# carlozamu/dynamic-video-compression-surveillance

Hardware: AMD Instinct MI355X
Metric: Mpixels/s (frames/s × H×W) 1080p frame-diff path @1/2/4/8 GPU; % HBM roofline (higher is better)
Workload: dtype u8; 1 GPU; fd_1080p_single_feed_per_gpu; width=1920, height=1080, feeds_per_gpu=1, io=device, ring_frames=384, noisy=False, in_format=BGR, out_format=BGR, launch=batched, frames_per_launch=383, output_sets=2, parallelism=feed-per-gpu x1

## Files before the change

dynamic-video-compression-surveillance_amd/_native.py:

```python
from __future__ import annotations

import ctypes
import glob
import os
import shutil
import subprocess

PKG_DIR = os.path.dirname(os.path.abspath(__file__))
CSRC = os.path.join(PKG_DIR, "csrc")
LIB_PATH = os.path.join(PKG_DIR, "libdvc_hip.so")
HIPCC_FLAGS = ["--offload-arch=gfx950", "-O3", "-std=c++17", "-fPIC", "-shared", "-ffp-contract=off"]

DVC_OK = 0
DVC_E_INVALID, DVC_E_HIP, DVC_E_STATE, DVC_E_NOMEM, DVC_E_UNSUPPORTED = -1, -2, -3, -4, -5
DVC_E_ODD_DCT = -6
DVC_FLAG_DEVICE_PTRS = 0x1
DVC_FLAG_KTIMING = 0x2
DVC_FLAG_KEEP_PLANES = 0x4
DVC_FLAG_JOIN_STREAM = 0x8
DVC_FLAG_OF_DIRECT_SUMS = 0x10
DVC_FLAG_OUT_I420 = 0x20
DVC_FLAG_FD_UNFUSED = 0x40
KTIME_OUT, KTIME_FRONT_FUSED = 0, 1
KTIME_FLOW, KTIME_FLOW_SCAN, KTIME_FLOW_SCAN2 = 2, 3, 4
FMT_BGR, FMT_I420, FMT_NV12 = 0, 1, 2
FMT_GRAY = 3
FORMATS = {"BGR": FMT_BGR, "I420": FMT_I420, "NV12": FMT_NV12}

PLANE_GRAY, PLANE_MOTION, PLANE_FILTERED, PLANE_ACC, PLANE_DILATED = range(5)
OF_PLANE_RAW, OF_PLANE_SMOOTH, OF_PLANE_MORPH, OF_PLANE_RECT, OF_PLANE_GRAY = range(5)

ABI_VERSION = 10
MAX_BATCH = 512


class DvcError(RuntimeError):

    def __init__(self, code: int, msg: str):
        super().__init__(f"dvc error {code}: {msg}")
        self.code = code


class FdParams(ctypes.Structure):
    _fields_ = [
        ("width", ctypes.c_int32),
# ... 470 lines not shown
```

dynamic-video-compression-surveillance_amd/csrc/fd_api.hip:

```cpp
#include <hip/hip_runtime.h>
#include <cstdlib>

#include <cmath>
#include <cstdio>
#include <algorithm>
#include <cstring>
#include <utility>
#include <vector>

#include "../../include/dvc.h"
#include "fd_kernels.h"
#include "klaunch.h"
#include "host_common.h"
#include "yuv_kernels.h"
#include "tune.h"

using dvc_host::fail;
using dvc_host::dct_matrix;
using dvc_host::gauss_taps;

struct FdGraph {
    std::vector<dvc::KNode> rec[4];
    std::vector<hipGraphNode_t> node[4];
    hipGraph_t g = nullptr;
// ... 397 lines not shown
    if (p.flags & DVC_FLAG_KEEP_PLANES) {
        if ((e = h->mem.alloc(&h->dbg_dil, 8 * H * WW)) != hipSuccess) return bad(e, "hipMalloc");
    }
    if (!(p.flags & DVC_FLAG_DEVICE_PTRS)) {
        const size_t Fi = (size_t)h->sip * h->sh * mb, Fo = 3 * N * (size_t)mb;
        for (Stage& st : h->stage) {
            if ((e = h->mem.alloc(&st.d_in, Fi)) != hipSuccess) return bad(e, "hipMalloc");
            if ((e = h->mem.alloc(&st.d_ov, Fo)) != hipSuccess) return bad(e, "hipMalloc");
            if ((e = h->mem.alloc(&st.d_cp, Fo)) != hipSuccess) return bad(e, "hipMalloc");
            if ((e = h->mem.alloc_pinned(&st.h_in, Fi)) != hipSuccess) return bad(e, "hipHostMalloc");
            if ((e = h->mem.alloc_pinned(&st.h_ov, Fo)) != hipSuccess) return bad(e, "hipHostMalloc");
            if ((e = h->mem.alloc_pinned(&st.h_cp, Fo)) != hipSuccess) return bad(e, "hipHostMalloc");
            for (hipEvent_t* ev : {&st.ev_h2d, &st.ev_d2h, &st.ev_free})
                if ((e = h->mem.event(ev)) != hipSuccess) return bad(e, "hipEventCreate");
        }
        if ((e = h->mem.alloc_pinned(&h->h_acc, N)) != hipSuccess) return bad(e, "hipHostMalloc");
    }
    if ((e = hipMemsetAsync(h->stats, 0, 8 * 4 * 64, h->stream)) != hipSuccess) return bad(e, "hipMemset");
    if ((e = hipMemsetAsync(h->err, 0xff, 8, h->stream)) != hipSuccess) return bad(e, "hipMemset");
    if ((e = hipMemsetAsync(h->acc, 0, accb, h->stream)) != hipSuccess) return bad(e, "hipMemset");
    {
        size_t sz[dvc::CclBufs::NARR];
        dvc::CclBufs::sizes(h->g, mb, sz);
        if ((e = hipMemsetAsync(h->slot[0].c.gpar, 0, sz[6], h->stream)) != hipSuccess) return bad(e, "hipMemset");
    }
    if ((e = hipStreamSynchronize(h->stream)) != hipSuccess) return bad(e, "hipStreamSynchronize");
    *out = h;
    return DVC_OK;
}

}

static int stage_input(dvc_fd* h, Slot& S, const uint8_t* src, size_t pitch, size_t fstride, int n,
                       const uint8_t** d, int* dp, size_t* dfs, int crows, dvc::SrcFmt* sf)
{
    if (sf) *sf = dvc::SrcFmt{DVC_FMT_BGR, 0, 0, 0};
    const int direct = in_place(h, src, pitch, fstride, n);
    if (direct == 1) {
        *d = src;
        *dp = (int)pitch;
        *dfs = fstride;
        return DVC_OK;
    }
    if (sf && direct == 2) {
        const dvc::YuvLayout L = dvc::yuv_layout(src, pitch, h->fmt, crows, fstride);
        *sf = dvc::SrcFmt{h->fmt, L.uoff, L.voff, L.cpitch};
        *d = src;
// ... 96 lines not shown
{
    if (n <= S.gc_frames) return DVC_OK;
    int cap = 1;
    while (cap < n) cap *= 2;
    cap = std::min(cap, std::min(h->max_batch, GRAPH_OWN_CCL_FRAMES));
    if (!S.gc_mem.dev.empty()) {
        if (S.recorded) HIP_OK(hipEventSynchronize(S.ev_out));
        S.gc_mem.free_all();
        S.gc_frames = 0;
    }
    size_t sz[dvc::CclBufs::NARR];
    dvc::CclBufs::sizes(h->g, cap, sz);
    S.gc = S.c;
    void** ptrs[dvc::CclBufs::NARR];
    S.gc.ptrs(ptrs);
    for (int i = 0; i < dvc::CclBufs::NARR; ++i) {
        if (!dvc::CclBufs::working_set(i)) continue;
        const hipError_t e = S.gc_mem.alloc(ptrs[i], sz[i]);
        if (e != hipSuccess) {
            S.gc_mem.free_all();
            return dvc_host::create_failed(e, "graph contour-filter set");
        }
    }
    HIP_OK(hipMemsetAsync(S.gc.gpar, 0, sz[6], graph_stream(h, (int)(&S - h->slot))));
    S.gc_frames = cap;
    return DVC_OK;
}

static int enqueue_graph(dvc_fd* h, Slot& S, std::vector<dvc::KNode> (&rec)[4], const std::vector<hipEvent_t>& wait_out,
                         bool shared)
{
    const int k = (int)(h->seq % NSLOT);
    Slot& P = h->slot[(h->seq + NSLOT - 1) % NSLOT];
    hipStream_t z = graph_stream(h, k);
    const hipEvent_t ccl_ev = P.recorded && P.graph && !P.shared_ccl ? P.ev_acc : P.ev_ccl;
    FdGraph* G = nullptr;
    for (FdGraph& x : S.graphs) {
        bool same = x.shared == shared;
        for (int sg = 0; sg < 4 && same; ++sg) {
            same = x.rec[sg].size() == rec[sg].size();
            for (size_t u = 0; same && u < rec[sg].size(); ++u) same = x.rec[sg][u].same_shape(rec[sg][u]);
        }
        if (same) {
            G = &x;
            break;
        }
    }
// ... 202 lines not shown
    a.n = n;
    a.ksize = h->p.ksize;
    a.anchor = h->p.anchor;
    a.alpha = h->p.alpha;
    a.beta = h->p.beta;
    a.gamma = h->p.gamma;
    a.quant = h->p.quant;
    a.qinv = 1.0 / (double)h->p.quant;
    {
        const float z = std::rint(std::fmaf(0.0f, h->p.alpha, std::fmaf(0.0f, h->p.beta, h->p.gamma)));
        a.acc0_fixed = z < 0.5f && z > -0.5f;
        const float dil1 = std::fmaf(255.0f, h->p.beta, h->p.gamma);
        static const bool acc_general = dvc::tune_env("DVC_ACC_GENERAL") != nullptr;
        a.acc_fast = dvc::acc_fast_ok(h->p.alpha, h->p.beta, h->p.gamma) && !acc_general;
        std::memcpy(&a.dil1_bits, &dil1, 4);
    }
    a.M = h->M;
    a.Mtab = h->Mtab;
    a.stats = h->stats;
    a.dbg_dil = h->dbg_dil;
    a.err = h->err;
    a.frame0 = h->frames;
    h->last_fused = fused;
    if (graph) {
        std::vector<dvc::KNode> rec[4];
        hipError_t e[4];
        hipStream_t z = graph_stream(h, (int)(h->seq % NSLOT));
        const bool shared = n > GRAPH_OWN_CCL_FRAMES;
        if (!shared) {
            rc = graph_ccl(h, S, n);
            if (rc) return rc;
        }
        dvc::g_krec = &rec[0];
        e[0] = dvc::launch_front(d, dp, dfs, sf, n, h->gray[h->gcur], h->gray[h->gcur ^ 1], h->gs, S.c.mbits, h->g,
                                 h->p.ithresh, z, fused ? &fo : nullptr);
        dvc::g_krec = &rec[1];
        e[1] = dvc::launch_ccl(shared ? S.c : S.gc, h->g, n, h->p.min_area2, z);
        dvc::g_krec = &rec[2];
        e[2] = dvc::launch_accumulate(a, z);
        dvc::g_krec = &rec[3];
        e[3] = dvc::launch_out(a, z, fused);
        dvc::g_krec = nullptr;
        for (hipError_t x : e) HIP_OK(x);
        rc = enqueue_graph(h, S, rec, wait_out, shared);
        if (rc) return rc;
        h->prev_graph = true;
        S.graph = true;
        S.shared_ccl = shared;
    } else {
        if (timed) {
            while (h->ev.size() < h->ev_used + 2) {
                hipEvent_t e;
                HIP_OK(hipEventCreate(&e));
                h->ev.push_back(e);
            }
        }
        if (timed && fused) HIP_OK(hipEventRecord(h->ev[h->ev_used], h->s_front));
        if (!(skip & 1))
            HIP_OK(dvc::launch_front(d, dp, dfs, sf, n, h->gray[h->gcur], h->gray[h->gcur ^ 1], h->gs, S.c.mbits, h->g,
                                     h->p.ithresh, h->s_front, fused ? &fo : nullptr));
        if (timed && fused) {
            HIP_OK(hipEventRecord(h->ev[h->ev_used + 1], h->s_front));
            h->ev_used += 2;
        }
        HIP_OK(hipEventRecord(S.ev_front, h->s_front));
        HIP_OK(hipStreamWaitEvent(s_ccl, S.ev_front, 0));
        if (S.recorded) HIP_OK(hipStreamWaitEvent(s_ccl, S.ev_acc, 0));
        if (!(skip & 2)) HIP_OK(dvc::launch_ccl(S.c, h->g, n, h->p.min_area2, s_ccl));
        HIP_OK(hipEventRecord(S.ev_ccl, s_ccl));
        HIP_OK(hipStreamWaitEvent(h->s_acc, S.ev_ccl, 0));
        if (S.recorded) HIP_OK(hipStreamWaitEvent(h->s_acc, S.ev_out, 0));
        if (!(skip & 4)) HIP_OK(dvc::launch_accumulate(a, h->s_acc));
        HIP_OK(hipEventRecord(S.ev_acc, h->s_acc));
        HIP_OK(hipStreamWaitEvent(h->s_out, S.ev_acc, 0));
        if (timed && !fused) HIP_OK(hipEventRecord(h->ev[h->ev_used], h->s_out));
        if (!(skip & 8)) HIP_OK(dvc::launch_out(a, h->s_out, fused));
        if (timed && !fused) {
            HIP_OK(hipEventRecord(h->ev[h->ev_used + 1], h->s_out));
            h->ev_used += 2;
        }
        HIP_OK(hipEventRecord(S.ev_out, h->s_out));
        h->prev_graph = false;
        S.graph = false;
        S.shared_ccl = true;
    }
    h->gcur ^= 1;
    S.recorded = true;
    h->seq++;
    h->frames += (uint64_t)n;
    h->last_n = n;
    return DVC_OK;
}

static int drain_stage(dvc_fd* h, Stage& st)
{
// ... 212 lines not shown
    if (width < 4 || height < 4 || width > 65520)
        return fail(DVC_E_INVALID, "mask %dx%d: sides must be 4..65520", width, height);
    HIP_OK(hipSetDevice(device));
    dvc::RowGeom g{width, height, (width + 63) / 64, width / 2 + 1};
    const size_t W = width, H = height, WW = g.WW;
    std::vector<uint64_t> bits(H * WW, 0);
    for (size_t y = 0; y < H; ++y)
        for (size_t x = 0; x < W; ++x)
            if (mask[y * W + x]) bits[y * WW + x / 64] |= 1ull << (x % 64);
    dvc::CclBufs c{};
    size_t sz[dvc::CclBufs::NARR];
    void** ptrs[dvc::CclBufs::NARR];
    dvc::CclBufs::sizes(g, 1, sz);
    c.ptrs(ptrs);
    unsigned long long* stats = nullptr;
    dvc_host::DevMem mem;
    hipError_t e = mem.alloc(&stats, 8 * 4 * 64);
    for (int i = 0; i < dvc::CclBufs::NARR && e == hipSuccess; ++i) e = mem.alloc(ptrs[i], sz[i]);
    if (e != hipSuccess) return fail(DVC_E_NOMEM, "hipMalloc failed");
    c.stats = stats;
    hipStream_t s = nullptr;
    e = hipMemcpy(c.mbits, bits.data(), 8 * H * WW, hipMemcpyHostToDevice);
    if (e == hipSuccess) e = hipMemset(stats, 0, 8 * 4 * 64);
    if (e == hipSuccess) e = hipMemset(c.gpar, 0, sz[6]);
    if (e == hipSuccess) e = dvc::launch_ccl(c, g, 1, min_area2, s);
    if (e == hipSuccess) e = hipDeviceSynchronize();
    unsigned long long st[4];
    if (e == hipSuccess) e = dvc_host::fold_stats(stats, st);
    if (e == hipSuccess) e = dvc_host::read_bit_plane(c.kbits, W, H, WW, filtered);
    if (e != hipSuccess) return fail(DVC_E_HIP, "contour filter: %s", hipGetErrorString(e));
    if (components) *components = st[2];
    return DVC_OK;
}

}
```

dynamic-video-compression-surveillance_amd/csrc/fd_kernels.h:

```cpp
#pragma once
#include <hip/hip_runtime.h>
#include <stdint.h>

namespace dvc {

struct RowGeom {
    int W, H;
    int WW;
    int CAP;
};

struct GaussTaps {
    int n;
    uint16_t t[64];
};

struct alignas(8) DctMat {
    float m[64];
    float mt[64];
};

struct CclBufs {
    uint64_t* mbits;
    uint64_t* fbits;
    uint16_t *rs, *re;
    uint32_t* nfg;
    uint32_t* fpar;
    uint32_t* gpar;
    uint8_t* gE;
    uint32_t* area2;
    uint64_t* kbits;
    unsigned long long* stats;
    uint8_t* kocc = nullptr;
    int kfull = 0;
    uint32_t* rowb = nullptr;
    static size_t rowb_bytes(const RowGeom& g, size_t frames) { return (size_t)8 * g.H * frames; }

    __host__ __device__ static size_t bits_per_frame(const RowGeom& g) { return (size_t)g.H * g.WW; }
    __host__ __device__ CclBufs frame(size_t f, const RowGeom& g) const
    {
        const size_t nb = (size_t)g.H * g.WW, nr = (size_t)g.H * g.CAP, ng = (size_t)g.H * (g.CAP + 1);
        return CclBufs{mbits + f * nb, fbits + f * nb, rs + f * nr, re + f * nr, nfg + f * g.H, fpar + f * nr,
                       gpar + f * (ng + 1), gE + f * ng, area2 + f * nr, kbits + f * nb, stats,
                       kocc ? kocc + f * g.H : nullptr, kfull, rowb + f * 2 * g.H};
    }
    static constexpr int NARR = 11;
    static void sizes(const RowGeom& g, size_t frames, size_t out[NARR])
    {
        const size_t nb = (size_t)g.H * g.WW, nr = (size_t)g.H * g.CAP, ng = (size_t)g.H * (g.CAP + 1);
        const size_t s[NARR] = {8 * nb, 8 * nb, 2 * nr, 2 * nr, 4 * (size_t)g.H, 4 * nr, 4 * (ng + 1), ng, 4 * nr, 8 * nb,
                                rowb_bytes(g, 1)};
        for (int i = 0; i < NARR; ++i) out[i] = s[i] * frames;
    }
    void ptrs(void** out[NARR])
    {
        void** p[NARR] = {(void**)&mbits, (void**)&fbits, (void**)&rs,    (void**)&re,    (void**)&nfg, (void**)&fpar,
                          (void**)&gpar,  (void**)&gE,    (void**)&area2, (void**)&kbits, (void**)&rowb};
        for (int i = 0; i < NARR; ++i) out[i] = p[i];
    }
    static bool working_set(int i) { return (i >= 1 && i <= 8) || i == 10; }
};

struct SrcFmt {
    int fmt;
    size_t uoff, voff, cpitch;
};

struct BackArgs {
    RowGeom g;
    const uint8_t* bgr;
    int pitch;
    size_t fstride;
    SrcFmt sf;
    uint8_t* acc;
    int ap;
    uint8_t* overlay;
    uint8_t* compressed;
    int opitch;
    size_t ostride;
    int obytes;
    int out_i420;
    const uint64_t* kbits;
    const uint8_t* kocc;
// ... 32 lines not shown
    size_t ostride;
    float quant;
    double qinv;
    DctMat M;
    int B;
    int i420;
};
hipError_t launch_front(const uint8_t* bgr, int pitch, size_t fstride, const SrcFmt& sf, int n, const uint8_t* gray_in,
                        uint8_t* gray_out, int gs, uint64_t* mbits, const RowGeom& g, int ithresh, hipStream_t s,
                        const FrontOut* fo = nullptr);
struct ResizeTab {
    int sw, sh, dw, dh;
    int area2x;
    int simd_end;
    const int* xo;
    const int* yo;
};
void resize_tables(int sw, int sh, int dw, int dh, int* host_x , int* host_y , int* area2x,
                   int* simd_end);
hipError_t launch_resize(const uint8_t* src, int spitch, size_t sstride, uint8_t* dst, int dpitch, size_t dstride,
                         int n, const ResizeTab& t, hipStream_t s);
int band_rows(const RowGeom& g);
size_t ccl_max_lds(const RowGeom& g);
hipError_t launch_ccl(const CclBufs& c, const RowGeom& g, int n, int64_t min_area2, hipStream_t s);
hipError_t launch_accumulate(const BackArgs& a, hipStream_t s);
inline bool acc_fast_ok(float alpha, float beta, float gamma)
{
    const float d0 = __builtin_fmaf(0.0f, beta, gamma), d1 = __builtin_fmaf(255.0f, beta, gamma);
    uint32_t d0b;
    __builtin_memcpy(&d0b, &d0, 4);
    return d0b == 0 && alpha >= 0.0f && alpha <= 1.0f && d1 >= 0.0f && d1 <= 255.0f &&
           __builtin_rintf(__builtin_fmaf(255.0f, alpha, d1)) <= 255.0f;
}
hipError_t launch_out(const BackArgs& a, hipStream_t s, bool fix = false);
inline bool fast_block(int B) { return B == 4 || B == 8; }

}
```

dynamic-video-compression-surveillance_amd/csrc/fd_kernels.hip:

```cpp
#include <hip/hip_runtime.h>
#include <stdint.h>

#include <algorithm>
#include <cmath>
#include <cstdlib>
#include <cstring>

#include "dvc_device.h"
#include "fd_kernels.h"
#include "klaunch.h"
#include "dct_const.h"
#include "yuv_px.h"
#include "../../include/dvc.h"
#include "tune.h"

namespace dvc {

thread_local std::vector<KNode>* g_krec = nullptr;

__global__ void __launch_bounds__(256) k_gray(const uint8_t* __restrict__ bgr, int pitch,
                                              uint8_t* __restrict__ gray, int W, int H, int gs)
{
    int q = blockIdx.x * 256 + threadIdx.x;
    int y = blockIdx.y;
// ... 763 lines not shown
        const uint32_t base = fb.rowb[2 * y];
        const uint8_t* ge = gE + (fb.rowb[2 * y + 1] - 1);
        for (int k = sl; k < n; k += CG) {
            const uint32_t root = fpar[base + k];
            if (!((int64_t)area2[root] > min_area2)) continue;
            const int e = re[base + k];
            paint_bits(s_k, 0, g.WW, rs[base + k], e);
            if (k + 1 < n && !ge[k + 1]) paint_bits(s_k, 0, g.WW, e + 1, (int)rs[base + k + 1] - 1);
        }
    }
    wave_sync_lds();
    unsigned long long any = 0;
    if (act)
        for (int w = sl; w < g.WW; w += CG) any |= s_k[w];
    for (int d = 1; d < CG; d <<= 1) any |= __shfl_xor(any, d, CG);
    if (act && (any || !fb.kocc || fb.kfull))
        for (int w = sl; w < g.WW; w += CG) kbits[(size_t)y * g.WW + w] = s_k[w];
    if (act && sl == 0 && fb.kocc) fb.kocc[y] = any ? 1 : 0;
}

template <int CG>
__global__ void __launch_bounds__(256) k_resolve(CclBufs cb, RowGeom g)
{
    const CclBufs fb = cb.frame(blockIdx.y, g);
    const uint16_t* __restrict__ rs = fb.rs;
    const uint16_t* __restrict__ re = fb.re;
    const uint32_t* __restrict__ nfg = fb.nfg;
    uint32_t* fpar = fb.fpar;
    uint32_t* gpar = fb.gpar;
    uint8_t* __restrict__ gE = fb.gE;
    const uint64_t* __restrict__ mbits = fb.mbits;
    uint64_t* __restrict__ fbits = fb.fbits;
    extern __shared__ __attribute__((aligned(16))) unsigned long long lds_r[];
    const int slot = threadIdx.x / CG, sl = threadIdx.x & (CG - 1);
    const int y = blockIdx.x * cg_rows<CG>() + slot;
    const bool act = y < g.H;
    unsigned long long* s_f = lds_r + (size_t)slot * g.WW;
    const int n = act ? (int)nfg[y] : 0;
    if (n)
        for (int w = sl; w < g.WW; w += CG) s_f[w] = mbits[(size_t)y * g.WW + w];
    wave_sync_lds();
    if (n) {
        const uint32_t base = fb.rowb[2 * y], gbase = fb.rowb[2 * y + 1];
        for (int k = sl; k <= n; k += CG) {
            const int a = k == 0 ? 0 : (int)re[base + k - 1] + 1;
            const int b = k == n ? g.W - 1 : (int)rs[base + k] - 1;
            uint8_t e = 1;
            if (a <= b) {
                const uint32_t r = uf_find(gpar, gbase + k);
                atomicMin(gpar + gbase + k, r);
                e = r == 0;
                if (!e) {
                    uf_union(fpar, base + k - 1, base + k);
                    paint_bits(s_f, 0, g.WW, a, b);
                }
            }
            gE[gbase - 1 + k] = e;
        }
    }
    wave_sync_lds();
    if (n)
        for (int w = sl; w < g.WW; w += CG) fbits[(size_t)y * g.WW + w] = s_f[w];
}

template <int CG>
__global__ void __launch_bounds__(256) k_area(CclBufs cb, RowGeom g)
{
    const CclBufs fb = cb.frame(blockIdx.y, g);
    const uint16_t* __restrict__ rs = fb.rs;
    const uint16_t* __restrict__ re = fb.re;
    const uint32_t* __restrict__ nfg = fb.nfg;
    uint32_t* fpar = fb.fpar;
    const uint8_t* __restrict__ gE = fb.gE;
    const uint64_t* __restrict__ fbits = fb.fbits;
    uint32_t* __restrict__ area2 = fb.area2;
    unsigned long long* __restrict__ stats = fb.stats;
    extern __shared__ __attribute__((aligned(16))) unsigned long long lds_b[];
    const int lane = threadIdx.x & 63;
    const int slot = threadIdx.x / CG, sl = threadIdx.x & (CG - 1), g0 = lane & ~(CG - 1);
    const int y = blockIdx.x * cg_rows<CG>() + slot;
    const bool act = y < g.H;
    unsigned long long* s_b = lds_b + (size_t)slot * g.WW;
    const bool last = y == g.H - 1;
    const int n = act ? (int)nfg[y] : 0;
    const bool fnext = n && !last && nfg[y + 1];
    if (n)
        for (int w = sl; w < g.WW; w += CG) s_b[w] = fnext ? fbits[(size_t)(y + 1) * g.WW + w] : 0ull;
    wave_sync_lds();
    int comps = 0;
    if (act) {
        const uint32_t base = fb.rowb[2 * y];
        const uint8_t* ge = gE + (fb.rowb[2 * y + 1] - 1);
        const uint64_t* b = reinterpret_cast<const uint64_t*>(s_b);
        const unsigned long long gmask = ((1ull << CG) - 1ull) << g0;
        for (int k0 = 0; k0 < n; k0 += CG) {
            const int k = k0 + sl;
            const bool valid = k < n;
            const uint32_t id = base + (valid ? k : 0);
            uint32_t r = 0xffffffffu;
            int c = 0;
            if (valid) {
                r = uf_find(fpar, id);
                atomicMin(fpar + id, r);
                comps += r == id;
            }
            if (valid && !last) {
                int s = rs[id], e = re[id];
                c = 2 * popc_range(b, s, e);
                if (k == 0 || ge[k]) {
                    int bs = bit_at(b, s);
                    c -= bs;
                    if (s >= 1 && bs && bit_at(b, s - 1)) c += 1;
                }
                if (k == n - 1 || ge[k + 1]) {
                    int be = bit_at(b, e);
                    c -= be;
                    if (e <= g.W - 2 && be && bit_at(b, e + 1)) c += 1;
                }
                if (k + 1 < n && !ge[k + 1]) c += 2 * popc_range(b, e + 1, (int)rs[id + 1] - 1);
            }
            const uint32_t rp = __shfl_up(r, 1, CG);
            const bool head = sl == 0 || rp != r;
            const unsigned long long heads = __ballot(head) & gmask;
            const unsigned long long after = heads & (lane == 63 ? 0ull : (~0ull << (lane + 1)));
            const int seg_end = after ? __builtin_ctzll(after) - 1 : g0 + CG - 1;
            const int incl = group_incl_scan<CG>(c);
            const int seg = __shfl(incl, seg_end, 64) - incl + c;
            if (head && valid && seg) atomicAdd(area2 + r, (uint32_t)seg);
        }
    }
    for (int d = 32; d >= 1; d >>= 1) comps += __shfl_xor(comps, d, 64);
    if (lane == 0 && comps) atomicAdd(stats + STAT_SLOT(blockIdx.x) * 4 + 2, (unsigned long long)comps);
}

template <int B> struct BlkT;
template <> struct BlkT<4> { typedef uint16_t T; };
template <> struct BlkT<8> { typedef uint64_t T; };

template <int B>
__global__ void __launch_bounds__(256) k_dilate(BackArgs a)
{
    typedef typename BlkT<B>::T BT;
// ... 57 lines not shown
            }
        }
    };
    if (R <= 64) rows(std::false_type{});
    else rows(std::true_type{});
#pragma unroll
    for (int i = 0; i < B; ++i)
        if (y0 + i >= H) out[i] = 0;
    if (a.dbg_dil && t == a.n - 1) {
#pragma unroll
        for (int i = 0; i < B; ++i)
            if (y0 + i < H) a.dbg_dil[(size_t)(y0 + i) * WW + wi] = out[i];
    }
    uint8_t* db = reinterpret_cast<uint8_t*>(a.dblk) + (size_t)t * NBY * NBX * sizeof(BT);
    constexpr int PER = 64 / B;
    const int nb = min(PER, NBX - wi * PER);
    const uint32_t dbo = (uint32_t)(by * NBX + wi * PER) * (uint32_t)sizeof(BT);
#pragma unroll
    for (int b = 0; b < PER; ++b) {
        uint64_t f = 0;
#pragma unroll
        for (int i = 0; i < B; ++i) f |= ((out[i] >> (B * b)) & ((1ull << B) - 1)) << (B * i);
        if (b < nb) *reinterpret_cast<BT*>(db + (dbo + (uint32_t)(b * sizeof(BT)))) = (BT)f;
    }
}

__device__ __forceinline__ uint32_t hibits16(const uint32_t (&w)[4])
{
    auto pm = [](uint32_t x, unsigned short k) { return as_u32(as_u16x2(x) * (u16x2)k); };
    uint32_t y[4];
#pragma unroll
    for (int k = 0; k < 4; ++k) y[k] = pm(w[k] & 0x80808080u, 0x81);
    const uint32_t z01 = __builtin_amdgcn_perm(y[1], y[0], 0x07050301u);
    const uint32_t z23 = __builtin_amdgcn_perm(y[3], y[2], 0x07050301u);
    const uint32_t v = __builtin_amdgcn_perm(pm(z23, 0x41), pm(z01, 0x41), 0x07050301u);
    return __builtin_amdgcn_perm(0u, pm(v, 0x11), 0x04040301u);
}

template <int B, bool FAST>
__global__ void __launch_bounds__(64) k_acc(BackArgs a)
{
    typedef typename BlkT<B>::T BT;
    constexpr BT ROWM = (BT)((1u << B) - 1);
    const int lane = threadIdx.x;
    const int NBX = a.NBX, NBY = a.NBY, AP = a.ap;
    const int bxi = blockIdx.x * 64 + lane, by = blockIdx.y;
// ... 768 lines not shown
    while (x <= w - 16) x += 16;
    while (x < w - 8) x += 8;
    *simd_end = x;
}

hipError_t launch_resize(const uint8_t* src, int spitch, size_t sstride, uint8_t* dst, int dpitch, size_t dstride,
                         int n, const ResizeTab& t, hipStream_t s)
{
    klaunch(k_resize, dim3((t.dw + 255) / 256, t.dh, n), dim3(256), 0, s, src, spitch, sstride, dst, dpitch,
                       dstride, t);
    return hipGetLastError();
}

size_t band_lds(const RowGeom& g, int bh, int budget)
{
    return (size_t)16 * bh * g.WW + (size_t)4 * bh * (g.WW + 1) + 8 + (size_t)4 * budget;
}

int band_rows(const RowGeom&) { return BAND_ROWS; }

size_t ccl_max_lds(const RowGeom& g)
{
    return std::max({band_lds(g, BAND_ROWS, 1024), (size_t)8 * merge_lds_words(g.WW) * (256 / MG),
                     (size_t)8 * g.WW * cg_rows<8>()});
}

static int band_budget(const RowGeom& g)
{
    static const int kb = [] { const char* e = dvc::tune_env("DVC_BAND_LDS_KB"); return e ? std::max(8, atoi(e)) : 0; }();
    const long long rest = kb * 1024LL - (long long)band_lds(g, BAND_ROWS, 0);
    return (int)std::max<long long>(1024, rest / 4);
}

hipError_t launch_ccl(const CclBufs& c, const RowGeom& g, int n, int64_t min_area2, hipStream_t s)
{
    if (!c.rowb) return hipErrorInvalidValue;
    static const int sub = [] {
        const char* e = dvc::tune_env("DVC_CCL_SUB");
        return e ? atoi(e) : 0;
    }();
    if (sub > 0 && n > sub) {
        for (int f0 = 0; f0 < n; f0 += sub) {
            const hipError_t e = launch_ccl(c.frame(f0, g), g, std::min(sub, n - f0), min_area2, s);
            if (e != hipSuccess) return e;
        }
        return hipSuccess;
    }
    const int BH = band_rows(g), nb = (g.H + BH - 1) / BH, budget = band_budget(g);
    klaunch(k_band, dim3(nb, n), dim3(BAND_NT), band_lds(g, BH, budget), s, c, g, budget);
    if (nb > 1)
        klaunch(k_merge, dim3((nb - 1 + 256 / MG - 1) / (256 / MG), n), dim3(256),
                           8 * merge_lds_words(g.WW) * (256 / MG), s, c, g, BH);
    static const int cg_env = [] { const char* e = dvc::tune_env("DVC_CCL_CG"); return e ? atoi(e) : 0; }();
    const int cg = cg_env == 8 || cg_env == 16 ? cg_env : ((long long)n * g.H >= 96LL * 1080 ? 8 : 16);
    if (cg == 8) {
        const int grows = (g.H + cg_rows<8>() - 1) / cg_rows<8>();
        const size_t glds = (size_t)8 * g.WW * cg_rows<8>();
        klaunch(k_resolve<8>, dim3(grows, n), dim3(256), glds, s, c, g);
        klaunch(k_area<8>, dim3(grows, n), dim3(256), glds, s, c, g);
        klaunch(k_paint<8>, dim3(grows, n), dim3(256), glds, s, c, g, min_area2);
    } else {
        const int grows = (g.H + cg_rows<16>() - 1) / cg_rows<16>();
        const size_t glds = (size_t)8 * g.WW * cg_rows<16>();
        klaunch(k_resolve<16>, dim3(grows, n), dim3(256), glds, s, c, g);
        klaunch(k_area<16>, dim3(grows, n), dim3(256), glds, s, c, g);
        klaunch(k_paint<16>, dim3(grows, n), dim3(256), glds, s, c, g, min_area2);
    }
    return hipGetLastError();
}

template <int B>
static hipError_t launch_acc(const BackArgs& a, hipStream_t s)
{
    klaunch(k_dilate<B>, dim3((a.g.WW * a.NBY + 255) / 256, a.n), dim3(256), 0, s, a);
    if (a.acc_fast)
        klaunch((k_acc<B, true>), dim3(a.SW, a.NBY), dim3(64), 0, s, a);
    else
        klaunch((k_acc<B, false>), dim3(a.SW, a.NBY), dim3(64), 0, s, a);
    return hipGetLastError();
}

hipError_t launch_accumulate(const BackArgs& a, hipStream_t s)
{
    if (a.B == 4) return launch_acc<4>(a, s);
    if (a.B == 8) return launch_acc<8>(a, s);
    klaunch(k_dilate_rows, dim3((a.g.WW * a.g.H + 255) / 256, a.n), dim3(256), 0, s, a);
    klaunch(k_acc_rows, dim3(a.g.WW, a.g.H), dim3(64), 0, s, a);
    return hipGetLastError();
}

static void launch_gen(const BackArgs& a, int rx0, int rx1, int ry0, int ry1, int jbx, int jby, int fast, hipStream_t s)
{
    if (rx0 >= rx1 || ry0 >= ry1) return;
    GenRegion R{rx0, rx1, ry0, ry1, std::max(1, std::min(jbx, rx1 - rx0)), std::max(1, std::min(jby, ry1 - ry0)), 0};
    R.njx = (rx1 - rx0 + R.jbx - 1) / R.jbx;
    const int njy = (ry1 - ry0 + R.jby - 1) / R.jby;
    const size_t lds = (size_t)8 * R.jbx * R.jby * a.B * a.B + (size_t)4 * R.jbx * R.jby;
    klaunch(k_out_gen, dim3(R.njx * njy, a.n), dim3(256), lds, s, a, R, fast);
}

hipError_t launch_out(const BackArgs& a, hipStream_t s, bool fix)
{
    const int B = a.B;
    if ((B == 4 && !dct4_is_const(a.M)) || (B == 8 && !dct8_is_const(a.M)))
        return hipErrorInvalidValue;
    const int per = std::max(1, 1024 / (B * B));
    if (!fast_block(B)) {
        int jb = 1;
// ... 55 lines not shown
```

dynamic-video-compression-surveillance_amd/fd.py:

```python
from __future__ import annotations

import ctypes
import math

import numpy as np

from . import _buffers as B
from . import _native as N
from ._worker import Worker


def derive_params(width: int, height: int, block_size: int = 4, motion_threshold: float = 0.5,
                  min_area: float = 500, kernel_size: int = 7, release_factor: float = 0.5,
                  quantization_level: float = 100, flags: int = 0, src_width: int = 0,
                  src_height: int = 0, in_format: str = "BGR", chroma_rows: int = 0) -> N.FdParams:
    p = N.FdParams()
    p.width, p.height = int(width), int(height)
    p.block = int(block_size)
    p.ithresh = max(-1, min(255, math.floor(motion_threshold)))
    p.min_area2 = math.floor(2.0 * float(min_area))
    p.ksize = int(kernel_size)
    p.anchor = int(kernel_size) // 2
    p.alpha = float(release_factor)
    p.beta = float(1 - release_factor)
    p.gamma = 0.0
    p.quant = float(quantization_level)
    p.prime_ksize = 25
    p.prime_sigma = 30.0
    p.flags = flags
    p.src_width, p.src_height = int(src_width or 0), int(src_height or 0)
    p.in_format = N.FORMATS[in_format]
    p.chroma_rows = int(chroma_rows)
    return p


class FDWorker(Worker):
    _abi, _destroy = "dvc_fd", "dvc_fd_destroy"
    _outs = ("overlay", "compressed")

    def __init__(self, width: int, height: int, *, device: int = 0, stream=None,
                 device_ptrs: bool = False, keep_planes: bool = False, ktiming: bool = False,
                 max_batch: int = 1, out_format: str = "BGR", fused: bool = True, **kwargs):
        if out_format not in ("BGR", "I420"):
            raise ValueError(f"out_format {out_format!r}: BGR or I420")
        flags = (N.DVC_FLAG_OUT_I420 if out_format == "I420" else 0) | (0 if fused else N.DVC_FLAG_FD_UNFUSED)
        self.out_format = out_format
        W, H = int(width), int(height)
        self.SW = int(kwargs.get("src_width") or width)
        self.SH = int(kwargs.get("src_height") or height)
        self._oshape = (H, W, 3) if out_format == "BGR" else (H * 3 // 2, W)
        self._open(derive_params(width, height, flags=flags, **kwargs), kwargs.get("in_format", "BGR"),
                   (self.SW, self.SH), (self._oshape, self._oshape), device=device, stream=stream,
                   device_ptrs=device_ptrs, keep_planes=keep_planes, ktiming=ktiming, max_batch=max_batch)

    def set_state(self, prev_gray, acc) -> None:
        g = np.ascontiguousarray(prev_gray, dtype=np.uint8)
        a = np.ascontiguousarray(acc, dtype=np.uint8)
        if g.shape != (self.H, self.W) or a.shape != (self.H, self.W):
            raise ValueError(f"state planes must be ({self.H}, {self.W})")
        N.check(self._lib.dvc_fd_set_state(self._h, g.ctypes.data, a.ctypes.data))

    def step(self, frame, overlay=None, compressed=None, acc=None, want=("overlay", "compressed")):
        if acc is not None:
            if self.device_ptrs:
                acc = B.device_buf(acc, (self.H, self.W), self.device, "acc", batched=False)[0]
            else:
                acc = B.host_out(acc, (self.H, self.W), "acc", False).ctypes.data
        return self._step(frame, overlay, compressed, want, acc)
# ... 17 lines not shown
```

include/dvc.h:

```cpp
#ifndef DVC_H
#define DVC_H

#include <stddef.h>
#include <stdint.h>

#ifdef __cplusplus
extern "C" {
#endif

#define DVC_ABI_VERSION 10
#define DVC_MAX_BATCH 512

#define DVC_OK             0
#define DVC_E_INVALID     -1
#define DVC_E_HIP         -2
#define DVC_E_STATE       -3
#define DVC_E_NOMEM       -4
#define DVC_E_UNSUPPORTED -5
#define DVC_E_ODD_DCT     -6

#define DVC_FLAG_DEVICE_PTRS 0x1u
#define DVC_FLAG_KTIMING     0x2u
#define DVC_FLAG_KEEP_PLANES 0x4u
#define DVC_FLAG_JOIN_STREAM 0x8u
#define DVC_FLAG_OF_DIRECT_SUMS 0x10u
#define DVC_FLAG_OUT_I420    0x20u

#define DVC_FLAG_FD_UNFUSED  0x40u

#define DVC_FMT_BGR  0
#define DVC_FMT_I420 1
#define DVC_FMT_NV12 2
#define DVC_FMT_GRAY 3

int dvc_yuv420_to_bgr(const uint8_t* yuv, size_t pitch, int fmt, int chroma_rows, int width, int height, int n,
                      size_t frame_stride, uint8_t* bgr, size_t bgr_pitch, size_t bgr_stride, int device,
                      void* hip_stream, uint32_t flags);
int dvc_bgr_to_i420(const uint8_t* bgr, size_t bgr_pitch, size_t bgr_stride, int width, int height, int n,
                    uint8_t* yuv, size_t pitch, int chroma_rows, size_t frame_stride, int device, void* hip_stream,
                    uint32_t flags);


typedef struct dvc_fd_params {
    int32_t width;
    int32_t height;
    int32_t block;
    int32_t ithresh;
    int64_t min_area2;
    int32_t ksize;
    int32_t anchor;
    float alpha;
// ... 194 lines not shown
```

Baseline: 407,800 Mpixels/s.

## Fuse kept-pixel paint with block dilation and move run area into resolve

```diff
diff --git a/dynamic-video-compression-surveillance_amd/_native.py b/dynamic-video-compression-surveillance_amd/_native.py
--- a/dynamic-video-compression-surveillance_amd/_native.py
+++ b/dynamic-video-compression-surveillance_amd/_native.py
@@ -21,6 +21,7 @@
 DVC_FLAG_OF_DIRECT_SUMS = 0x10
 DVC_FLAG_OUT_I420 = 0x20
 DVC_FLAG_FD_UNFUSED = 0x40
+DVC_FLAG_FD_KEPT_PLANE = 0x80
 KTIME_OUT, KTIME_FRONT_FUSED = 0, 1
 KTIME_FLOW, KTIME_FLOW_SCAN, KTIME_FLOW_SCAN2 = 2, 3, 4
 FMT_BGR, FMT_I420, FMT_NV12 = 0, 1, 2
diff --git a/dynamic-video-compression-surveillance_amd/csrc/fd_api.hip b/dynamic-video-compression-surveillance_amd/csrc/fd_api.hip
--- a/dynamic-video-compression-surveillance_amd/csrc/fd_api.hip
+++ b/dynamic-video-compression-surveillance_amd/csrc/fd_api.hip
@@ -443,7 +443,7 @@
     {
         size_t sz[dvc::CclBufs::NARR];
         dvc::CclBufs::sizes(h->g, mb, sz);
-        if ((e = hipMemsetAsync(h->slot[0].c.gpar, 0, sz[6], h->stream)) != hipSuccess) return bad(e, "hipMemset");
+        if ((e = hipMemsetAsync(h->slot[0].c.gpar, 0, sz[dvc::CclBufs::I_GPAR], h->stream)) != hipSuccess) return bad(e, "hipMemset");
     }
     if ((e = hipStreamSynchronize(h->stream)) != hipSuccess) return bad(e, "hipStreamSynchronize");
     *out = h;
@@ -586,7 +586,7 @@
             return dvc_host::create_failed(e, "graph contour-filter set");
         }
     }
-    HIP_OK(hipMemsetAsync(S.gc.gpar, 0, sz[6], graph_stream(h, (int)(&S - h->slot))));
+    HIP_OK(hipMemsetAsync(S.gc.gpar, 0, sz[dvc::CclBufs::I_GPAR], graph_stream(h, (int)(&S - h->slot))));
     S.gc_frames = cap;
     return DVC_OK;
 }
@@ -835,6 +835,7 @@
     a.err = h->err;
     a.frame0 = h->frames;
     h->last_fused = fused;
+    const bool onchip = !(h->p.flags & DVC_FLAG_FD_KEPT_PLANE) && dvc::fuse_paint_dilate(S.c, a);
     if (graph) {
         std::vector<dvc::KNode> rec[4];
         hipError_t e[4];
@@ -848,9 +849,9 @@
         e[0] = dvc::launch_front(d, dp, dfs, sf, n, h->gray[h->gcur], h->gray[h->gcur ^ 1], h->gs, S.c.mbits, h->g,
                                  h->p.ithresh, z, fused ? &fo : nullptr);
         dvc::g_krec = &rec[1];
-        e[1] = dvc::launch_ccl(shared ? S.c : S.gc, h->g, n, h->p.min_area2, z);
+        e[1] = dvc::launch_ccl(shared ? S.c : S.gc, h->g, n, h->p.min_area2, z, onchip ? &a : nullptr);
         dvc::g_krec = &rec[2];
-        e[2] = dvc::launch_accumulate(a, z);
+        e[2] = dvc::launch_accumulate(a, z, onchip);
         dvc::g_krec = &rec[3];
         e[3] = dvc::launch_out(a, z, fused);
         dvc::g_krec = nullptr;
@@ -879,11 +880,11 @@
         HIP_OK(hipEventRecord(S.ev_front, h->s_front));
         HIP_OK(hipStreamWaitEvent(s_ccl, S.ev_front, 0));
         if (S.recorded) HIP_OK(hipStreamWaitEvent(s_ccl, S.ev_acc, 0));
-        if (!(skip & 2)) HIP_OK(dvc::launch_ccl(S.c, h->g, n, h->p.min_area2, s_ccl));
+        if (!(skip & 2)) HIP_OK(dvc::launch_ccl(S.c, h->g, n, h->p.min_area2, s_ccl, onchip ? &a : nullptr));
         HIP_OK(hipEventRecord(S.ev_ccl, s_ccl));
         HIP_OK(hipStreamWaitEvent(h->s_acc, S.ev_ccl, 0));
         if (S.recorded) HIP_OK(hipStreamWaitEvent(h->s_acc, S.ev_out, 0));
-        if (!(skip & 4)) HIP_OK(dvc::launch_accumulate(a, h->s_acc));
+        if (!(skip & 4)) HIP_OK(dvc::launch_accumulate(a, h->s_acc, onchip));
         HIP_OK(hipEventRecord(S.ev_acc, h->s_acc));
         HIP_OK(hipStreamWaitEvent(h->s_out, S.ev_acc, 0));
         if (timed && !fused) HIP_OK(hipEventRecord(h->ev[h->ev_used], h->s_out));
@@ -1142,7 +1143,7 @@
     hipStream_t s = nullptr;
     e = hipMemcpy(c.mbits, bits.data(), 8 * H * WW, hipMemcpyHostToDevice);
     if (e == hipSuccess) e = hipMemset(stats, 0, 8 * 4 * 64);
-    if (e == hipSuccess) e = hipMemset(c.gpar, 0, sz[6]);
+    if (e == hipSuccess) e = hipMemset(c.gpar, 0, sz[dvc::CclBufs::I_GPAR]);
     if (e == hipSuccess) e = dvc::launch_ccl(c, g, 1, min_area2, s);
     if (e == hipSuccess) e = hipDeviceSynchronize();
     unsigned long long st[4];
diff --git a/dynamic-video-compression-surveillance_amd/csrc/fd_kernels.h b/dynamic-video-compression-surveillance_amd/csrc/fd_kernels.h
--- a/dynamic-video-compression-surveillance_amd/csrc/fd_kernels.h
+++ b/dynamic-video-compression-surveillance_amd/csrc/fd_kernels.h
@@ -22,7 +22,6 @@
 
 struct CclBufs {
     uint64_t* mbits;
-    uint64_t* fbits;
     uint16_t *rs, *re;
     uint32_t* nfg;
     uint32_t* fpar;
@@ -40,25 +39,26 @@
     __host__ __device__ CclBufs frame(size_t f, const RowGeom& g) const
     {
         const size_t nb = (size_t)g.H * g.WW, nr = (size_t)g.H * g.CAP, ng = (size_t)g.H * (g.CAP + 1);
-        return CclBufs{mbits + f * nb, fbits + f * nb, rs + f * nr, re + f * nr, nfg + f * g.H, fpar + f * nr,
+        return CclBufs{mbits + f * nb, rs + f * nr, re + f * nr, nfg + f * g.H, fpar + f * nr,
                        gpar + f * (ng + 1), gE + f * ng, area2 + f * nr, kbits + f * nb, stats,
                        kocc ? kocc + f * g.H : nullptr, kfull, rowb + f * 2 * g.H};
     }
-    static constexpr int NARR = 11;
+    static constexpr int NARR = 10;
+    static constexpr int I_GPAR = 5;
     static void sizes(const RowGeom& g, size_t frames, size_t out[NARR])
     {
         const size_t nb = (size_t)g.H * g.WW, nr = (size_t)g.H * g.CAP, ng = (size_t)g.H * (g.CAP + 1);
-        const size_t s[NARR] = {8 * nb, 8 * nb, 2 * nr, 2 * nr, 4 * (size_t)g.H, 4 * nr, 4 * (ng + 1), ng, 4 * nr, 8 * nb,
+        const size_t s[NARR] = {8 * nb, 2 * nr, 2 * nr, 4 * (size_t)g.H, 4 * nr, 4 * (ng + 1), ng, 4 * nr, 8 * nb,
                                 rowb_bytes(g, 1)};
         for (int i = 0; i < NARR; ++i) out[i] = s[i] * frames;
     }
     void ptrs(void** out[NARR])
     {
-        void** p[NARR] = {(void**)&mbits, (void**)&fbits, (void**)&rs,    (void**)&re,    (void**)&nfg, (void**)&fpar,
+        void** p[NARR] = {(void**)&mbits, (void**)&rs,    (void**)&re,    (void**)&nfg,   (void**)&fpar,
                           (void**)&gpar,  (void**)&gE,    (void**)&area2, (void**)&kbits, (void**)&rowb};
         for (int i = 0; i < NARR; ++i) out[i] = p[i];
     }
-    static bool working_set(int i) { return (i >= 1 && i <= 8) || i == 10; }
+    static bool working_set(int i) { return (i >= 1 && i <= 7) || i == 9; }
 };
 
 struct SrcFmt {
@@ -137,8 +137,10 @@
                          int n, const ResizeTab& t, hipStream_t s);
 int band_rows(const RowGeom& g);
 size_t ccl_max_lds(const RowGeom& g);
-hipError_t launch_ccl(const CclBufs& c, const RowGeom& g, int n, int64_t min_area2, hipStream_t s);
-hipError_t launch_accumulate(const BackArgs& a, hipStream_t s);
+bool fuse_paint_dilate(const CclBufs& c, const BackArgs& a);
+hipError_t launch_ccl(const CclBufs& c, const RowGeom& g, int n, int64_t min_area2, hipStream_t s,
+                      const BackArgs* back = nullptr);
+hipError_t launch_accumulate(const BackArgs& a, hipStream_t s, bool dilated = false);
 inline bool acc_fast_ok(float alpha, float beta, float gamma)
 {
     const float d0 = __builtin_fmaf(0.0f, beta, gamma), d1 = __builtin_fmaf(255.0f, beta, gamma);
diff --git a/dynamic-video-compression-surveillance_amd/csrc/fd_kernels.hip b/dynamic-video-compression-surveillance_amd/csrc/fd_kernels.hip
--- a/dynamic-video-compression-surveillance_amd/csrc/fd_kernels.hip
+++ b/dynamic-video-compression-surveillance_amd/csrc/fd_kernels.hip
@@ -809,6 +809,7 @@
 template <int CG>
 __global__ void __launch_bounds__(256) k_resolve(CclBufs cb, RowGeom g)
 {
+    constexpr int ROWS = cg_rows<CG>();
     const CclBufs fb = cb.frame(blockIdx.y, g);
     const uint16_t* __restrict__ rs = fb.rs;
     const uint16_t* __restrict__ re = fb.re;
@@ -817,68 +818,83 @@
     uint32_t* gpar = fb.gpar;
     uint8_t* __restrict__ gE = fb.gE;
     const uint64_t* __restrict__ mbits = fb.mbits;
-    uint64_t* __restrict__ fbits = fb.fbits;
+    uint32_t* __restrict__ area2 = fb.area2;
     extern __shared__ __attribute__((aligned(16))) unsigned long long lds_r[];
+    const int WW = g.WW;
     const int slot = threadIdx.x / CG, sl = threadIdx.x & (CG - 1);
-    const int y = blockIdx.x * cg_rows<CG>() + slot;
+    const int y = blockIdx.x * ROWS + slot, yh = (blockIdx.x + 1) * ROWS;
     const bool act = y < g.H;
-    unsigned long long* s_f = lds_r + (size_t)slot * g.WW;
+    unsigned long long* s_f = lds_r + (size_t)slot * WW;
+    unsigned long long* s_h = lds_r + (size_t)ROWS * WW;
     const int n = act ? (int)nfg[y] : 0;
-    if (n)
-        for (int w = sl; w < g.WW; w += CG) s_f[w] = mbits[(size_t)y * g.WW + w];
-    wave_sync_lds();
-    if (n) {
-        const uint32_t base = fb.rowb[2 * y], gbase = fb.rowb[2 * y + 1];
-        for (int k = sl; k <= n; k += CG) {
-            const int a = k == 0 ? 0 : (int)re[base + k - 1] + 1;
-            const int b = k == n ? g.W - 1 : (int)rs[base + k] - 1;
-            uint8_t e = 1;
-            if (a <= b) {
-                const uint32_t r = uf_find(gpar, gbase + k);
-                atomicMin(gpar + gbase + k, r);
-                e = r == 0;
-                if (!e) {
-                    uf_union(fpar, base + k - 1, base + k);
-                    paint_bits(s_f, 0, g.WW, a, b);
-                }
-            }
-            gE[gbase - 1 + k] = e;
-        }
-    }
-    wave_sync_lds();
-    if (n)
-        for (int w = sl; w < g.WW; w += CG) fbits[(size_t)y * g.WW + w] = s_f[w];
+    const int nh = yh < g.H ? (int)nfg[yh] : 0;
+    for (int w = sl; w < WW; w += CG) s_f[w] = n ? mbits[(size_t)y * WW + w] : 0ull;
+    for (int w = threadIdx.x; w < WW; w += 256) s_h[w] = nh ? mbits[(size_t)yh * WW + w] : 0ull;
+    __syncthreads();
+    const uint32_t base = n ? fb.rowb[2 * y] : 0u, gbase = n ? fb.rowb[2 * y + 1] : 0u;
+    const uint32_t hbase = nh ? fb.rowb[2 * yh] : 0u, hgbase = nh ? fb.rowb[2 * yh + 1] : 0u;
+    const int hl = 255 - (int)threadIdx.x;
+    const int nown = n && sl <= n ? (n - sl) / CG + 1 : 0;
+    const int nhalo = nh && hl <= nh ? (nh - hl) / 256 + 1 : 0;
+    for (int it = 0; it < nown + nhalo; ++it) {
+        const bool halo = it >= nown;
+        const int k = halo ? hl + (it - nown) * 256 : sl + it * CG;
+        const int nn = halo ? nh : n;
+        const uint32_t bs = halo ? hbase : base, gb = halo ? hgbase : gbase;
+        const int a = k == 0 ? 0 : (int)re[bs + k - 1] + 1;
+        const int b = k == nn ? g.W - 1 : (int)rs[bs + k] - 1;
+        uint8_t e = 1;
+        if (a <= b) {
+            const uint32_t r = uf_find(gpar, gb + k);
+            if (!halo) atomicMin(gpar + gb + k, r);
+            e = r == 0;
+            if (!e) {
+                if (!halo) uf_union(fpar, bs + k - 1, bs + k);
+                paint_bits(halo ? s_h : s_f, 0, WW, a, b);
+            }
+        }
+        if (!halo) gE[gb - 1 + k] = e;
+    }
+    __syncthreads();
+    if (!n || y == g.H - 1) return;
+    const uint64_t* f = reinterpret_cast<const uint64_t*>(s_f);
+    const uint64_t* b = reinterpret_cast<const uint64_t*>(slot + 1 < ROWS ? s_f + WW : s_h);
+    for (int k = sl; k < n; k += CG) {
+        const uint32_t id = base + k;
+        const int s = rs[id], e = re[id];
+        const bool hole_l = k > 0 && bit_at(f, s - 1), hole_r = k < n - 1 && bit_at(f, e + 1);
+        int c = 2 * popc_range(b, s, e);
+        if (!hole_l) {
+            int bs = bit_at(b, s);
+            c -= bs;
+            if (s >= 1 && bs && bit_at(b, s - 1)) c += 1;
+        }
+        if (!hole_r) {
+            int be = bit_at(b, e);
+            c -= be;
+            if (e <= g.W - 2 && be && bit_at(b, e + 1)) c += 1;
+        }
+        if (hole_r) c += 2 * popc_range(b, e + 1, (int)rs[id + 1] - 1);
+        area2[id] = (uint32_t)c;
+    }
 }
 
 template <int CG>
 __global__ void __launch_bounds__(256) k_area(CclBufs cb, RowGeom g)
 {
     const CclBufs fb = cb.frame(blockIdx.y, g);
-    const uint16_t* __restrict__ rs = fb.rs;
-    const uint16_t* __restrict__ re = fb.re;
     const uint32_t* __restrict__ nfg = fb.nfg;
     uint32_t* fpar = fb.fpar;
-    const uint8_t* __restrict__ gE = fb.gE;
-    const uint64_t* __restrict__ fbits = fb.fbits;
-    uint32_t* __restrict__ area2 = fb.area2;
+    uint32_t* area2 = fb.area2;
     unsigned long long* __restrict__ stats = fb.stats;
-    extern __shared__ __attribute__((aligned(16))) unsigned long long lds_b[];
     const int lane = threadIdx.x & 63;
     const int slot = threadIdx.x / CG, sl = threadIdx.x & (CG - 1), g0 = lane & ~(CG - 1);
     const int y = blockIdx.x * cg_rows<CG>() + slot;
     const bool act = y < g.H;
-    unsigned long long* s_b = lds_b + (size_t)slot * g.WW;
-    const bool last = y == g.H - 1;
     const int n = act ? (int)nfg[y] : 0;
-    const bool fnext = n && !last && nfg[y + 1];
-    if (n)
-        for (int w = sl; w < g.WW; w += CG) s_b[w] = fnext ? fbits[(size_t)(y + 1) * g.WW + w] : 0ull;
-    wave_sync_lds();
     int comps = 0;
-    if (act) {
+    if (n) {
         const uint32_t base = fb.rowb[2 * y];
-        const uint8_t* ge = gE + (fb.rowb[2 * y + 1] - 1);
-        const uint64_t* b = reinterpret_cast<const uint64_t*>(s_b);
         const unsigned long long gmask = ((1ull << CG) - 1ull) << g0;
         for (int k0 = 0; k0 < n; k0 += CG) {
             const int k = k0 + sl;
@@ -890,21 +906,7 @@
                 r = uf_find(fpar, id);
                 atomicMin(fpar + id, r);
                 comps += r == id;
-            }
-            if (valid && !last) {
-                int s = rs[id], e = re[id];
-                c = 2 * popc_range(b, s, e);
-                if (k == 0 || ge[k]) {
-                    int bs = bit_at(b, s);
-                    c -= bs;
-                    if (s >= 1 && bs && bit_at(b, s - 1)) c += 1;
-                }
-                if (k == n - 1 || ge[k + 1]) {
-                    int be = bit_at(b, e);
-                    c -= be;
-                    if (e <= g.W - 2 && be && bit_at(b, e + 1)) c += 1;
-                }
-                if (k + 1 < n && !ge[k + 1]) c += 2 * popc_range(b, e + 1, (int)rs[id + 1] - 1);
+                if (r != id) c = (int)area2[id];
             }
             const uint32_t rp = __shfl_up(r, 1, CG);
             const bool head = sl == 0 || rp != r;
@@ -1008,6 +1010,109 @@
 #pragma unroll
         for (int i = 0; i < B; ++i) f |= ((out[i] >> (B * b)) & ((1ull << B) - 1)) << (B * i);
         if (b < nb) *reinterpret_cast<BT*>(db + (dbo + (uint32_t)(b * sizeof(BT)))) = (BT)f;
+    }
+}
+
+constexpr int PD_ROWS = 32;
+__host__ __device__ constexpr size_t paint_dilate_lds(int WW, int k) { return (size_t)(PD_ROWS + k - 1) * (8 * WW + 4); }
+
+template <int B, int CG>
+__global__ void __launch_bounds__(256) k_paint_dilate(CclBufs cb, BackArgs a, int64_t min_area2)
+{
+    typedef typename BlkT<B>::T BT;
+    constexpr int BRG = PD_ROWS / B, PER = 64 / B;
+    const RowGeom g = a.g;
+    const int W = g.W, H = g.H, WW = g.WW, NBX = a.NBX, NBY = a.NBY, t = blockIdx.y;
+    const int k = a.ksize, an = a.anchor, R = B + k - 1, NR = PD_ROWS + k - 1;
+    const CclBufs fb = cb.frame(t, g);
+    const uint16_t* __restrict__ rs = fb.rs;
+    const uint16_t* __restrict__ re = fb.re;
+    const uint32_t* __restrict__ nfg = fb.nfg;
+    const uint32_t* __restrict__ fpar = fb.fpar;
+    const uint8_t* __restrict__ gE = fb.gE;
+    const uint32_t* __restrict__ area2 = fb.area2;
+    extern __shared__ __attribute__((aligned(16))) unsigned long long lds_pd[];
+    unsigned long long* s_k = lds_pd;
+    uint32_t* s_any = reinterpret_cast<uint32_t*>(lds_pd + (size_t)NR * WW);
+    const int ytop = blockIdx.x * PD_ROWS - an;
+    for (int i = threadIdx.x; i < NR * WW; i += 256) s_k[i] = 0ull;
+    for (int i = threadIdx.x; i < NR; i += 256) s_any[i] = 0u;
+    __syncthreads();
+    const int slot = threadIdx.x / CG, sl = threadIdx.x & (CG - 1);
+    for (int lr = slot; lr < NR; lr += 256 / CG) {
+        const int y = ytop + lr;
+        if (y < 0 || y >= H) continue;
+        const int n = (int)nfg[y];
+        if (!n) continue;
+        const uint32_t base = fb.rowb[2 * y];
+        const uint8_t* ge = gE + (fb.rowb[2 * y + 1] - 1);
+        unsigned long long* row = s_k + (size_t)lr * WW;
+        for (int i = sl; i < n; i += CG) {
+            const uint32_t root = fpar[base + i];
+            if (!((int64_t)area2[root] > min_area2)) continue;
+            const int e = re[base + i];
+            paint_bits(row, 0, WW, rs[base + i], e);
+            if (i + 1 < n && !ge[i + 1]) paint_bits(row, 0, WW, e + 1, (int)rs[base + i + 1] - 1);
+            s_any[lr] = 1u;
+        }
+    }
+    __syncthreads();
+    const uint64_t* kb = reinterpret_cast<const uint64_t*>(s_k);
+    uint8_t* db = reinterpret_cast<uint8_t*>(a.dblk) + (size_t)t * NBY * NBX * sizeof(BT);
+    for (int idx = threadIdx.x; idx < WW * BRG; idx += 256) {
+        const int wi = idx % WW, byl = idx / WW, by = blockIdx.x * BRG + byl;
+        if (by >= NBY) break;
+        const int lr0 = byl * B;
+        uint32_t any = 0;
+        for (int r = 0; r < R; ++r) any |= s_any[lr0 + r];
+        if (wi == 0) a.docc[(size_t)by * a.n + t] = (uint8_t)(any != 0);
+        if (!any) continue;
+        const uint64_t vmask = (wi == WW - 1 && (W & 63)) ? (1ull << (W & 63)) - 1ull : ~0ull;
+        uint64_t out[B];
+#pragma unroll
+        for (int i = 0; i < B; ++i) out[i] = 0;
+        for (int r = 0; r < R; ++r) {
+            if (!s_any[lr0 + r]) continue;
+            const uint64_t* row = kb + (size_t)(lr0 + r) * WW;
+            const uint64_t c = row[wi], pv = wi > 0 ? row[wi - 1] : 0ull, nv = wi + 1 < WW ? row[wi + 1] : 0ull;
+            uint64_t o = c;
+            for (int off = 1; off <= k - 1 - an; ++off) o |= (c >> off) | (nv << (64 - off));
+            for (int off = 1; off <= an; ++off) o |= (c << off) | (pv >> (64 - off));
+            o &= vmask;
+#pragma unroll
+            for (int i = 0; i < B; ++i)
+                if (r - i >= 0 && r - i < k) out[i] |= o;
+        }
+#pragma unroll
+        for (int i = 0; i < B; ++i)
+            if (by * B + i >= H) out[i] = 0;
+        BT f[PER];
+#pragma unroll
+        for (int b = 0; b < PER; ++b) {
+            uint64_t v = 0;
+#pragma unroll
+            for (int i = 0; i < B; ++i) v |= ((out[i] >> (B * b)) & ((1ull << B) - 1)) << (B * i);
+            f[b] = (BT)v;
+        }
+        const int nb = min(PER, NBX - wi * PER);
+        uint8_t* dst = db + (size_t)(by * NBX + wi * PER) * sizeof(BT);
+        if (nb == PER && !(reinterpret_cast<uintptr_t>(dst) & 15)) {
+            constexpr int Q = 16 / (int)sizeof(BT);
+#pragma unroll
+            for (int q = 0; q < PER / Q; ++q) {
+                uint32_t d[4];
+#pragma unroll
+                for (int j = 0; j < 4; ++j) {
+                    if constexpr (B == 4) d[j] = (uint32_t)f[q * Q + 2 * j] | ((uint32_t)f[q * Q + 2 * j + 1] << 16);
+                    else d[j] = (uint32_t)((uint64_t)f[q * Q + (j >> 1)] >> (32 * (j & 1)));
+                }
+                *reinterpret_cast<uint4*>(dst + 16 * q) = make_uint4(d[0], d[1], d[2], d[3]);
+            }
+        } else {
+#pragma unroll
+            for (int b = 0; b < PER; ++b)
+                if (b < nb) reinterpret_cast<BT*>(dst)[b] = f[b];
+        }
     }
 }
 
@@ -1822,7 +1927,7 @@
 size_t ccl_max_lds(const RowGeom& g)
 {
     return std::max({band_lds(g, BAND_ROWS, 1024), (size_t)8 * merge_lds_words(g.WW) * (256 / MG),
-                     (size_t)8 * g.WW * cg_rows<8>()});
+                     (size_t)8 * g.WW * (cg_rows<8>() + 1)});
 }
 
 static int band_budget(const RowGeom& g)
@@ -1832,13 +1937,35 @@
     return (int)std::max<long long>(1024, rest / 4);
 }
 
-hipError_t launch_ccl(const CclBufs& c, const RowGeom& g, int n, int64_t min_area2, hipStream_t s)
-{
-    if (!c.rowb) return hipErrorInvalidValue;
+static int ccl_sub()
+{
     static const int sub = [] {
         const char* e = dvc::tune_env("DVC_CCL_SUB");
         return e ? atoi(e) : 0;
     }();
+    return sub;
+}
+
+bool fuse_paint_dilate(const CclBufs& c, const BackArgs& a)
+{
+    return fast_block(a.B) && a.B + a.ksize - 1 <= 64 && paint_dilate_lds(a.g.WW, a.ksize) <= 32768 && a.kocc &&
+           a.docc && !c.kfull && !a.dbg_dil && ccl_sub() <= 0;
+}
+
+template <int CG>
+static void launch_paint_dilate(const CclBufs& c, const BackArgs& a, int64_t min_area2, hipStream_t s)
+{
+    const dim3 grid((a.NBY * a.B + PD_ROWS - 1) / PD_ROWS, a.n);
+    const size_t lds = paint_dilate_lds(a.g.WW, a.ksize);
+    if (a.B == 4) klaunch((k_paint_dilate<4, CG>), grid, dim3(256), lds, s, c, a, min_area2);
+    else klaunch((k_paint_dilate<8, CG>), grid, dim3(256), lds, s, c, a, min_area2);
+}
+
+hipError_t launch_ccl(const CclBufs& c, const RowGeom& g, int n, int64_t min_area2, hipStream_t s, const BackArgs* back)
+{
+    if (!c.rowb) return hipErrorInvalidValue;
+    if (back && (!fuse_paint_dilate(c, *back) || back->n != n)) return hipErrorInvalidValue;
+    const int sub = ccl_sub();
     if (sub > 0 && n > sub) {
         for (int f0 = 0; f0 < n; f0 += sub) {
             const hipError_t e = launch_ccl(c.frame(f0, g), g, std::min(sub, n - f0), min_area2, s);
@@ -1856,23 +1983,25 @@
     if (cg == 8) {
         const int grows = (g.H + cg_rows<8>() - 1) / cg_rows<8>();
         const size_t glds = (size_t)8 * g.WW * cg_rows<8>();
-        klaunch(k_resolve<8>, dim3(grows, n), dim3(256), glds, s, c, g);
-        klaunch(k_area<8>, dim3(grows, n), dim3(256), glds, s, c, g);
-        klaunch(k_paint<8>, dim3(grows, n), dim3(256), glds, s, c, g, min_area2);
+        klaunch(k_resolve<8>, dim3(grows, n), dim3(256), glds + 8 * g.WW, s, c, g);
+        klaunch(k_area<8>, dim3(grows, n), dim3(256), 0, s, c, g);
+        if (back) launch_paint_dilate<8>(c, *back, min_area2, s);
+        else klaunch(k_paint<8>, dim3(grows, n), dim3(256), glds, s, c, g, min_area2);
     } else {
         const int grows = (g.H + cg_rows<16>() - 1) / cg_rows<16>();
         const size_t glds = (size_t)8 * g.WW * cg_rows<16>();
-        klaunch(k_resolve<16>, dim3(grows, n), dim3(256), glds, s, c, g);
-        klaunch(k_area<16>, dim3(grows, n), dim3(256), glds, s, c, g);
-        klaunch(k_paint<16>, dim3(grows, n), dim3(256), glds, s, c, g, min_area2);
+        klaunch(k_resolve<16>, dim3(grows, n), dim3(256), glds + 8 * g.WW, s, c, g);
+        klaunch(k_area<16>, dim3(grows, n), dim3(256), 0, s, c, g);
+        if (back) launch_paint_dilate<16>(c, *back, min_area2, s);
+        else klaunch(k_paint<16>, dim3(grows, n), dim3(256), glds, s, c, g, min_area2);
     }
     return hipGetLastError();
 }
 
 template <int B>
-static hipError_t launch_acc(const BackArgs& a, hipStream_t s)
-{
-    klaunch(k_dilate<B>, dim3((a.g.WW * a.NBY + 255) / 256, a.n), dim3(256), 0, s, a);
+static hipError_t launch_acc(const BackArgs& a, hipStream_t s, bool dilated)
+{
+    if (!dilated) klaunch(k_dilate<B>, dim3((a.g.WW * a.NBY + 255) / 256, a.n), dim3(256), 0, s, a);
     if (a.acc_fast)
         klaunch((k_acc<B, true>), dim3(a.SW, a.NBY), dim3(64), 0, s, a);
     else
@@ -1880,10 +2009,11 @@
     return hipGetLastError();
 }
 
-hipError_t launch_accumulate(const BackArgs& a, hipStream_t s)
-{
-    if (a.B == 4) return launch_acc<4>(a, s);
-    if (a.B == 8) return launch_acc<8>(a, s);
+hipError_t launch_accumulate(const BackArgs& a, hipStream_t s, bool dilated)
+{
+    if (a.B == 4) return launch_acc<4>(a, s, dilated);
+    if (a.B == 8) return launch_acc<8>(a, s, dilated);
+    if (dilated) return hipErrorInvalidValue;
     klaunch(k_dilate_rows, dim3((a.g.WW * a.g.H + 255) / 256, a.n), dim3(256), 0, s, a);
     klaunch(k_acc_rows, dim3(a.g.WW, a.g.H), dim3(64), 0, s, a);
     return hipGetLastError();
diff --git a/dynamic-video-compression-surveillance_amd/fd.py b/dynamic-video-compression-surveillance_amd/fd.py
--- a/dynamic-video-compression-surveillance_amd/fd.py
+++ b/dynamic-video-compression-surveillance_amd/fd.py
@@ -40,10 +40,12 @@
 
     def __init__(self, width: int, height: int, *, device: int = 0, stream=None,
                  device_ptrs: bool = False, keep_planes: bool = False, ktiming: bool = False,
-                 max_batch: int = 1, out_format: str = "BGR", fused: bool = True, **kwargs):
+                 max_batch: int = 1, out_format: str = "BGR", fused: bool = True, kept_plane: bool = False,
+                 **kwargs):
         if out_format not in ("BGR", "I420"):
             raise ValueError(f"out_format {out_format!r}: BGR or I420")
-        flags = (N.DVC_FLAG_OUT_I420 if out_format == "I420" else 0) | (0 if fused else N.DVC_FLAG_FD_UNFUSED)
+        flags = (N.DVC_FLAG_OUT_I420 if out_format == "I420" else 0) | (0 if fused else N.DVC_FLAG_FD_UNFUSED) | \
+            (N.DVC_FLAG_FD_KEPT_PLANE if kept_plane else 0)
         self.out_format = out_format
         W, H = int(width), int(height)
         self.SW = int(kwargs.get("src_width") or width)
diff --git a/include/dvc.h b/include/dvc.h
--- a/include/dvc.h
+++ b/include/dvc.h
@@ -27,6 +27,7 @@
 #define DVC_FLAG_OUT_I420    0x20u
 
 #define DVC_FLAG_FD_UNFUSED  0x40u
+#define DVC_FLAG_FD_KEPT_PLANE 0x80u
 
 #define DVC_FMT_BGR  0
 #define DVC_FMT_I420 1
```

Result: faster. 441,000 Mpixels/s (median of 6 runs) (+8.1%).
